# ev-hansen/Configurable-Spectrograms

Measured on NVIDIA B200. Metric: orbits/sec (whole box, device-timed), higher is better.
Workload: dtype f32

## Files before the change

configurable_spectrograms_b200/csrc/raster.cu:

```cuda
#include "common.cuh"

namespace {

constexpr int I_UNDER = 256, I_OVER = 257, I_BAD = 258;

template <typename T>
__device__ __forceinline__ T round_to(double v) {
  return (T)v;
}

template <typename T>
__device__ __forceinline__ T log10_d(T v);
template <>
__device__ __forceinline__ float log10_d<float>(float v) {
  return (float)log10((double)v);
}
template <>
__device__ __forceinline__ double log10_d<double>(double v) {
  return log10(v);
}

template <typename T>
__device__ __forceinline__ T substitute(T v, const csg_panel_norm& nm, bool log_scale) {
  if (log_scale) {
    if (!is_finite(v) || v <= T(0)) v = (T)nm.fill_lo;
  } else {
    if (is_nan(v)) v = (T)nm.fill_lo;
    if (v == (T)(-CUDART_INF)) v = (T)nm.fill_lo;
    if (v == (T)CUDART_INF) v = (T)nm.fill_hi;
  }
  return v;
}

template <typename T>
__device__ __forceinline__ int cmap_index_direct(T v, const csg_panel_norm& nm, bool log_scale) {
  if (nm.degenerate == 1) return 0;
  T x;
  if (log_scale) {
    const T t = log10_d<T>(v);
    x = (T)((double)t - nm.t_vmin);
    x = (T)((double)x / nm.t_range);
    if (!is_finite(x)) return I_BAD;
  } else {
    x = (T)((double)v - nm.t_vmin);
    x = (T)((double)x / nm.t_range);
  }
  T xa = mul_rn(x, T(256));
  if (xa == T(256)) xa = T(255);
  if (is_nan(xa)) return I_BAD;
  if (xa < T(0)) return I_UNDER;
  if (xa >= T(256)) return I_OVER;
  return (int)xa;
}

template <typename T>
__device__ __forceinline__ int monotone_code(T v, const csg_panel_norm& nm, bool log_scale) {
  const int idx = cmap_index_direct<T>(v, nm, log_scale);
  return idx == I_UNDER ? -1 : (idx == I_OVER ? 256 : idx);
}

constexpr int kThr = 257;
constexpr int kThrPitch = 264;

template <typename T>
__global__ void __launch_bounds__(288)
    panel_threshold_kernel(const csg_panel* __restrict__ panels, const csg_panel_norm* __restrict__ norms, int n_panels,
                           T* __restrict__ thresholds) {
  typedef typename Key<T>::U U;
  const int pi = blockIdx.x;
  const int k = threadIdx.x;
  if (k >= kThr) return;
  const csg_panel_norm nm = norms[pi];
  T* out = thresholds + (size_t)pi * kThrPitch;
  if (nm.status != CSG_NORM_OK || nm.degenerate != 0) {
    out[k] = (T)CUDART_INF;
    return;
  }
  const bool log_scale = panels[pi].log_scale != 0;
  const U dom_lo = log_scale ? Key<T>::key((T)0) + 1 : Key<T>::key((T)(-CUDART_INF));
  const U dom_hi = log_scale ? Key<T>::key((T)CUDART_INF) - 1 : Key<T>::key((T)CUDART_INF);
  auto code = [&](U key) { return monotone_code<T>(Key<T>::val(key), nm, log_scale); };
  const double frac = (double)k / 256.0;
  double guess = log_scale ? exp10(nm.t_vmin + frac * nm.t_range) : nm.t_vmin + frac * nm.t_range;
  T gT = (T)guess;
  if (is_nan(gT)) gT = T(1);
  U g = Key<T>::key(gT);
  if (g < dom_lo) g = dom_lo;
  if (g > dom_hi) g = dom_hi;
  U lo, hi;
  U step = 2;
  bool found = true;
  if (code(g) >= k) {
    hi = g;
    while (true) {
      if (hi == dom_lo) {
        lo = hi;
        break;
      }
      lo = (hi - dom_lo > step) ? hi - step : dom_lo;
      if (code(lo) < k) break;
      hi = lo;
      step <<= 2;
    }
  } else {
    lo = g;
    while (true) {
      if (lo == dom_hi) {
        found = false;
        break;
      }
      hi = (dom_hi - lo > step) ? lo + step : dom_hi;
      if (code(hi) >= k) break;
      lo = hi;
      step <<= 2;
    }
  }
  if (!found) {
    out[k] = (T)CUDART_INF;
    return;
  }
  while (hi - lo > 1) {
    const U mid = lo + ((hi - lo) >> 1);
    if (code(mid) >= k)
      hi = mid;
    else
      lo = mid;
  }
  out[k] = Key<T>::val(hi);
}

template <typename T>
__global__ void panel_prepare_kernel(const csg_panel* __restrict__ panels, int n_panels,
                                     const csg_region_stats* __restrict__ stats, const double* __restrict__ zvals,
                                     csg_panel_norm* __restrict__ norms) {
  const int i = blockIdx.x * blockDim.x + threadIdx.x;
  if (i >= n_panels) return;
  const csg_panel p = panels[i];
  const csg_region_stats own = stats[p.stat_region >= 0 ? p.stat_region : p.region];
  const csg_region_stats pct = stats[p.pct_region >= 0 ? p.pct_region : p.region];
  const double given_lo = (p.zmin_slot >= 0 && zvals) ? zvals[p.zmin_slot] : p.z_min;
  const double given_hi = (p.zmax_slot >= 0 && zvals) ? zvals[p.zmax_slot] : p.z_max;
  double zmin = is_nan(given_lo) ? pct.p_lo : given_lo;
  double zmax = is_nan(given_hi) ? pct.p_hi : given_hi;
  csg_panel_norm nm;
  nm.status = CSG_NORM_OK;
  nm.degenerate = 0;
  nm.c0 = nm.c1 = 0.f;
  if (p.log_scale) {
    const double safe = own.n_pos > 0 ? own.min_pos : 1e-10;
    double m = zmin;
    if (safe > m) m = safe;
    if (1e-10 > m) m = 1e-10;
    zmin = m;
    nm.vmin = zmin, nm.vmax = zmax;
    nm.fill_lo = (double)(T)zmin;
    nm.fill_hi = (double)(T)zmax;
    if (zmin > zmax) {
      nm.status = CSG_NORM_VMIN_GT_VMAX;
    } else if (zmin == zmax) {
      nm.degenerate = 1;
    }
    const double tlo = log10(zmin), thi = log10(zmax);
    nm.t_vmin = tlo;
    nm.t_range = thi - tlo;
    if (nm.status == CSG_NORM_OK && !nm.degenerate && !(is_finite(tlo) && is_finite(thi)))
      nm.status = CSG_NORM_INVALID;
  } else {
    nm.fill_lo = (double)(T)zmin;
    nm.fill_hi = (double)(T)zmax;
    if (!(is_finite(zmin) && is_finite(zmax) && zmax > zmin)) {
      double lo = CUDART_INF, hi = -CUDART_INF;
      bool any = false;
      if (own.fin_min <= own.fin_max) {
        lo = own.fin_min, hi = own.fin_max, any = true;
      }
      if ((own.n_nan > 0 || own.n_neginf > 0) && !is_nan(nm.fill_lo)) {
        lo = fmin(lo, nm.fill_lo), hi = fmax(hi, nm.fill_lo), any = true;
      }
      if (own.n_posinf > 0 && !is_nan(nm.fill_hi)) {
        lo = fmin(lo, nm.fill_hi), hi = fmax(hi, nm.fill_hi), any = true;
      }
      zmin = any ? lo : CUDART_NAN;
      zmax = any ? hi : CUDART_NAN;
    }
    nm.vmin = zmin, nm.vmax = zmax;
    nm.t_vmin = zmin;
    nm.t_range = zmax - zmin;
    if (zmin == zmax)
      nm.degenerate = 1;
    else if (zmin > zmax)
      nm.status = CSG_NORM_VMIN_GT_VMAX;
    else if (is_nan(zmin) || is_nan(zmax))
      nm.degenerate = 2;
  }
  nm.c1 = p.log_scale ? (float)(256.0 * 0.30102999566398120 / nm.t_range) : (float)(256.0 / nm.t_range);
  nm.c0 = (float)(-256.0 * nm.t_vmin / nm.t_range) + 1.0f;
  norms[i] = nm;
}

constexpr int kRasterThreads = 512;
constexpr int kPixPerThread = 16;
constexpr int kPixPerBlock = kRasterThreads * kPixPerThread;
constexpr int kRows = kThr + 2;
constexpr int kLutRows = 260;

__device__ __forceinline__ float fast_log2(float x) {
  float r;
  asm("lg2.approx.ftz.f32 %0, %1;" : "=f"(r) : "f"(x));
  return r;
}

__device__ __forceinline__ void lds(float& v, unsigned addr) { asm volatile("ld.shared.f32 %0, [%1];" : "=f"(v) : "r"(addr)); }
__device__ __forceinline__ void lds(double& v, unsigned addr) { asm volatile("ld.shared.f64 %0, [%1];" : "=d"(v) : "r"(addr)); }

template <typename T>
__device__ __noinline__ int recount(T v, int n, unsigned thr_col) {
  if (is_nan(v)) return 258;
  auto thr_at = [&](int row) -> T {
    T t;
    lds(t, thr_col + (unsigned)row * (32u * (unsigned)sizeof(T)));
    return t;
  };
  while (n > 0 && !(thr_at(n) <= v)) --n;
  while (n < kThr && thr_at(n + 1) <= v) ++n;
  return n;
}

template <bool B>
struct Flag {
  static constexpr bool value = B;
};

template <typename T>
constexpr size_t raster_smem_bytes() {
  return (size_t)kLutRows * 32 * sizeof(uint32_t) + (size_t)kRows * 32 * sizeof(T);
}

template <typename T>
__global__ void __launch_bounds__(kRasterThreads, sizeof(T) == 4 ? 3 : 2)
    rasterise_kernel(const T* __restrict__ mats, const csg_region* __restrict__ regions,
                     const int32_t* __restrict__ pool, const csg_panel* __restrict__ panels,
                     const csg_panel_norm* __restrict__ norms, int chunk_offset, int n_chunks,
                     const int32_t* __restrict__ block_panel, const T* __restrict__ thresholds,
                     const uint32_t* __restrict__ lut, uint32_t* __restrict__ rgba, uint16_t* __restrict__ index) {
  extern __shared__ __align__(16) unsigned char s_raw[];
  T* s_thr = reinterpret_cast<T*>(s_raw);
  uint32_t* s_lut = reinterpret_cast<uint32_t*>(s_raw + (size_t)kRows * 32 * sizeof(T));

  const int tid = threadIdx.x, lane = tid & 31;
  const int per = (n_chunks + (int)gridDim.x - 1) / (int)gridDim.x;
  const int c_begin = (int)blockIdx.x * per, c_end = min(n_chunks, c_begin + per);
  if (c_begin >= c_end) return;
  for (int w = tid; w < kLutRows * 32; w += kRasterThreads) {
    const int n = w >> 5;
    const int idx = n == 0 ? I_UNDER : (n == kThr ? I_OVER : (n <= 256 ? n - 1 : I_BAD));
    s_lut[w] = (lut && n < 259) ? __ldg(lut + idx) : 0u;
  }
  unsigned thr_col = (unsigned)__cvta_generic_to_shared(s_thr + lane);
  unsigned lut_col = (unsigned)__cvta_generic_to_shared(s_lut + lane);
  asm volatile("" : "+r"(thr_col), "+r"(lut_col));
  auto thr_at = [&](int row) -> T {
    T v;
    lds(v, thr_col + (unsigned)row * (32u * (unsigned)sizeof(T)));
    return v;
  };
  auto lut_at = [&](int row) -> uint32_t {
    uint32_t v;
    asm volatile("ld.shared.u32 %0, [%1];" : "=r"(v) : "r"(lut_col + (unsigned)row * 128u));
    return v;
  };

  int cur_panel = -1;
  bool skip = false, log_scale = false;
  int degenerate = 0;
  unsigned nt = 1, n_pix = 0;
  int first_block = 0, ld = 0, t0 = 0, rows_off = -1;
  long long out_off = 0;
  float c1 = 0.f, c0 = 0.f;
  T fill_lo = T(0), fill_hi = T(0);
  const T* mat = mats;
  const int32_t *cols = pool, *rows = pool;
  bool in_vec = false;

  for (int chunk = c_begin; chunk < c_end; ++chunk) {
    const int blk = chunk + chunk_offset;
    const int pi = __ldg(block_panel + blk);
    if (pi != cur_panel) {
      cur_panel = pi;
      const csg_panel* pn = panels + pi;
      const csg_region* rg = regions + __ldg(&pn->region);
      const csg_panel_norm* nm = norms + pi;
      skip = __ldg(&nm->status) != CSG_NORM_OK;
      degenerate = __ldg(&nm->degenerate);
      log_scale = __ldg(&pn->log_scale) != 0;
      nt = (unsigned)__ldg(&rg->nt);
      n_pix = (unsigned)__ldg(&rg->ne) * nt;
      first_block = __ldg(&pn->first_block);
      out_off = __ldg(&pn->out_off);
      c1 = __ldg(&nm->c1), c0 = __ldg(&nm->c0);
      fill_lo = (T)__ldg(&nm->fill_lo), fill_hi = (T)__ldg(&nm->fill_hi);
      mat = mats + __ldg(&rg->mat_off);
      cols = pool + __ldg(&rg->cols_off);
      rows_off = __ldg(&rg->rows_off);
      rows = pool + (rows_off < 0 ? 0 : rows_off);
      ld = __ldg(&rg->ld), t0 = __ldg(&rg->t0);
      in_vec = sizeof(T) == 4 && rows_off < 0 && (ld & 3) == 0 && (__ldg(&rg->mat_off) & 3) == 0 &&
               (reinterpret_cast<uintptr_t>(mats) & 15) == 0;
      __syncthreads();
      if (!skip && degenerate == 0) {
        const T* thr = thresholds + (size_t)pi * kThrPitch;
        for (int w = tid; w < kRows * 32; w += kRasterThreads) {
          const int k = (w >> 5) - 1;
          s_thr[w] = k < 0 ? (T)(-CUDART_INF) : (k >= kThr ? (T)CUDART_INF : __ldg(thr + k));
        }
      }
      __syncthreads();
    }
    if (skip) continue;
    const unsigned first = (unsigned)(blk - first_block) * kPixPerBlock;
    const unsigned last = first + kPixPerBlock < n_pix ? first + kPixPerBlock : n_pix;
    uint32_t* out_rgba = rgba ? rgba + out_off : nullptr;
    uint16_t* out_idx = index ? index + out_off : nullptr;
    if (degenerate != 0) {
      const int idx = degenerate == 1 ? 0 : I_BAD;
      const int row = degenerate == 1 ? 1 : 258;
      for (unsigned i = first + tid; i < last; i += kRasterThreads) {
        if (out_rgba) out_rgba[i] = lut_at(row);
        if (out_idx) out_idx[i] = (uint16_t)idx;
      }
      continue;
    }

    auto substituted = [&](T v, auto log_c) -> T {
      constexpr bool LOG = decltype(log_c)::value;
      if (LOG) return (v > T(0)) & is_finite(v) ? v : fill_lo;
      v = (is_nan(v) || v == (T)(-CUDART_INF)) ? fill_lo : v;
      return (v == (T)CUDART_INF) ? fill_hi : v;
    };
    auto guess = [&](T v, auto log_c, bool& ok) -> int {
      constexpr bool LOG = decltype(log_c)::value;
      const float fv = (float)v;
      float gf = __fmaf_rn(LOG ? fast_log2(fv) : fv, c1, c0);
      gf = fminf(fmaxf(gf, 0.f), (float)kThr);
      const int n = (int)gf;
      const unsigned row = thr_col + (unsigned)n * (32u * (unsigned)sizeof(T));
      T lo_thr, hi_thr;
      lds(lo_thr, row);
      lds(hi_thr, row + 32u * (unsigned)sizeof(T));
      ok = ok & (lo_thr <= v) & !(hi_thr <= v);
      return n;
    };
    auto to_count = [&](T raw, auto log_c) -> int {
      const T v = substituted(raw, log_c);
      bool ok = true;
      const int n = guess(v, log_c, ok);
      return ok ? n : recount<T>(v, n, thr_col);
    };
    auto count_to_index = [](int n) -> int { return n == 0 ? I_UNDER : (n == kThr ? I_OVER : (n == 258 ? I_BAD : n - 1)); };

    const bool out_vec = (out_off & 3) == 0 && (!out_rgba || (reinterpret_cast<uintptr_t>(rgba) & 15) == 0) &&
                         (!out_idx || (reinterpret_cast<uintptr_t>(index) & 7) == 0);
    auto pixels = [&](auto log_c, auto rowlist_c, auto rgba_c, auto idx_c, auto vec_c) {
      constexpr bool ROWLIST = decltype(rowlist_c)::value;
      constexpr bool RGBA = decltype(rgba_c)::value, INDEX = decltype(idx_c)::value, VEC = decltype(vec_c)::value;
      constexpr unsigned G = 4, STEP = G * kRasterThreads;
      unsigned i = first + G * tid;
      unsigned j = i / nt, tt = i - j * nt;
      const unsigned dq = STEP / nt, dr = STEP - dq * nt;
      auto address = [&](unsigned jj, unsigned t) -> unsigned {
        return (unsigned)(__ldg(cols + jj) * ld + (ROWLIST ? __ldg(rows + t) : t0 + (int)t));
      };
      auto load4 = [&](unsigned jj, unsigned t, T* v) {
        if (t + (G - 1) < nt) {
          const unsigned a0 = address(jj, t);
          if (!ROWLIST && in_vec && (a0 & 3u) == 0) {
            if constexpr (sizeof(T) == 4) {
              const float4 q = __ldg(reinterpret_cast<const float4*>(mat + a0));
              v[0] = q.x, v[1] = q.y, v[2] = q.z, v[3] = q.w;
            }
          } else if (!ROWLIST) {
#pragma unroll
            for (unsigned u = 0; u < G; ++u) v[u] = __ldg(mat + a0 + u);
          } else {
            const unsigned c = (unsigned)(__ldg(cols + jj) * ld);
#pragma unroll
            for (unsigned u = 0; u < G; ++u) v[u] = __ldg(mat + c + __ldg(rows + t + u));
          }
        } else {
#pragma unroll
          for (unsigned u = 0; u < G; ++u) {
            v[u] = __ldg(mat + address(jj, t));
            if (++t == nt) t = 0, ++jj;
          }
        }
      };
      auto store4 = [&](unsigned at, const int* n) {
        if constexpr (RGBA) {
          if constexpr (VEC)
            *reinterpret_cast<uint4*>(out_rgba + at) = make_uint4(lut_at(n[0]), lut_at(n[1]), lut_at(n[2]), lut_at(n[3]));
          else {
#pragma unroll
            for (unsigned u = 0; u < G; ++u) out_rgba[at + u] = lut_at(n[u]);
          }
        }
        if constexpr (INDEX) {
          int idx[G];
#pragma unroll
          for (unsigned u = 0; u < G; ++u) idx[u] = count_to_index(n[u]);
          if constexpr (VEC)
            *reinterpret_cast<uint2*>(out_idx + at) =
                make_uint2((unsigned)idx[0] | ((unsigned)idx[1] << 16), (unsigned)idx[2] | ((unsigned)idx[3] << 16));
          else {
#pragma unroll
            for (unsigned u = 0; u < G; ++u) out_idx[at + u] = (uint16_t)idx[u];
          }
        }
      };
      auto advance = [&]() {
        i += STEP, j += dq, tt += dr;
        if (tt >= nt) tt -= nt, ++j;
      };
      auto classify_store = [&](unsigned at, T* v) {
        int x[G];
        bool ok = true;
#pragma unroll
        for (unsigned u = 0; u < G; ++u) {
          v[u] = substituted(v[u], log_c);
          x[u] = guess(v[u], log_c, ok);
        }
        if (!ok) {
#pragma unroll
          for (unsigned u = 0; u < G; ++u) x[u] = recount<T>(v[u], x[u], thr_col);
        }
        store4(at, x);
      };
      while (i + STEP + (G - 1) < last) {
        T a[G], b[G];
        const unsigned ia = i;
        load4(j, tt, a);
        advance();
        const unsigned ib = i;
        load4(j, tt, b);
        advance();
        classify_store(ia, a);
        classify_store(ib, b);
      }
      while (i + (G - 1) < last) {
        T cur[G];
        load4(j, tt, cur);
        classify_store(i, cur);
        advance();
      }
      if (i < last) {
        unsigned jj = j, t = tt;
        for (unsigned p = i; p < last; ++p) {
          const int n = to_count(__ldg(mat + address(jj, t)), log_c);
          if constexpr (RGBA) out_rgba[p] = lut_at(n);
          if constexpr (INDEX) out_idx[p] = (uint16_t)count_to_index(n);
          if (++t == nt) t = 0, ++jj;
        }
      }
    };
    auto by_output = [&](auto log_c, auto rowlist_c) {
      if (out_rgba && !out_idx && out_vec)
        pixels(log_c, rowlist_c, Flag<true>{}, Flag<false>{}, Flag<true>{});
      else if (out_rgba && out_idx && out_vec)
        pixels(log_c, rowlist_c, Flag<true>{}, Flag<true>{}, Flag<true>{});
      else if (out_rgba && out_idx)
        pixels(log_c, rowlist_c, Flag<true>{}, Flag<true>{}, Flag<false>{});
      else if (out_rgba)
        pixels(log_c, rowlist_c, Flag<true>{}, Flag<false>{}, Flag<false>{});
      else if (out_idx)
        pixels(log_c, rowlist_c, Flag<false>{}, Flag<true>{}, Flag<false>{});
    };
    if (log_scale) {
      if (rows_off < 0)
        by_output(Flag<true>{}, Flag<false>{});
      else
        by_output(Flag<true>{}, Flag<true>{});
    } else {
      if (rows_off < 0)
        by_output(Flag<false>{}, Flag<false>{});
      else
        by_output(Flag<false>{}, Flag<true>{});
    }
  }
}

}

extern "C" {

int32_t csg_raster_blocks(int32_t ne, int32_t nt) {
  if (ne <= 0 || nt <= 0) return 0;
  return (int32_t)(((long long)ne * nt + kPixPerBlock - 1) / kPixPerBlock);
}

size_t csg_threshold_bytes(int n_panels, int dtype) {
  return (size_t)(n_panels > 0 ? n_panels : 0) * kThrPitch * (dtype == CSG_F64 ? 8 : 4);
}

int csg_panel_prepare(csg_ctx* ctx, const csg_panel* d_panels, int n_panels, const csg_region* d_regions,
                      const csg_region_stats* d_stats, int dtype, const double* d_zvals, csg_panel_norm* d_norms,
                      void* d_thresholds) {
  (void)d_regions;
  if (!ctx) return CSG_ERR_ARG;
  if (n_panels <= 0) return CSG_OK;
  if (!d_panels || !d_stats || !d_norms || !d_thresholds) return csg_fail(ctx, CSG_ERR_ARG, "NULL argument");
  const int blocks = (n_panels + 127) / 128;
  if (dtype == CSG_F32) {
    panel_prepare_kernel<float><<<blocks, 128, 0, ctx->stream>>>(d_panels, n_panels, d_stats, d_zvals, d_norms);
    CSG_LAUNCH_CHECK(ctx, "panel_prepare_kernel");
    panel_threshold_kernel<float><<<n_panels, 288, 0, ctx->stream>>>(d_panels, d_norms, n_panels, (float*)d_thresholds);
  } else if (dtype == CSG_F64) {
    panel_prepare_kernel<double><<<blocks, 128, 0, ctx->stream>>>(d_panels, n_panels, d_stats, d_zvals, d_norms);
    CSG_LAUNCH_CHECK(ctx, "panel_prepare_kernel");
    panel_threshold_kernel<double><<<n_panels, 288, 0, ctx->stream>>>(d_panels, d_norms, n_panels, (double*)d_thresholds);
  } else {
    return csg_fail(ctx, CSG_ERR_ARG, "bad dtype %d", dtype);
  }
  CSG_LAUNCH_CHECK(ctx, "panel_threshold_kernel");
  return CSG_OK;
}

int csg_rasterise(csg_ctx* ctx, const void* d_mats, int dtype, const csg_region* d_regions,
                  const int32_t* d_index_pool, const csg_panel* d_panels, const csg_panel_norm* d_norms,
                  const void* d_thresholds, int n_panels, int total_blocks, int block_offset,
                  const int32_t* d_block_panel, const uint8_t* d_lut, uint8_t* d_rgba, uint16_t* d_index) {
  if (!ctx) return CSG_ERR_ARG;
  if (n_panels <= 0 || total_blocks <= 0) return CSG_OK;
  if (!d_mats || !d_regions || !d_index_pool || !d_panels || !d_norms || !d_thresholds || !d_block_panel)
    return csg_fail(ctx, CSG_ERR_ARG, "NULL argument");
  if (d_rgba && !d_lut) return csg_fail(ctx, CSG_ERR_ARG, "d_rgba requested without d_lut");
  static bool configured_dev[64] = {false};
  bool& configured = configured_dev[ctx->device & 63];
  if (!configured) {
    CSG_CUDA(ctx, cudaFuncSetAttribute(rasterise_kernel<float>, cudaFuncAttributeMaxDynamicSharedMemorySize,
                                       (int)raster_smem_bytes<float>()));
    CSG_CUDA(ctx, cudaFuncSetAttribute(rasterise_kernel<double>, cudaFuncAttributeMaxDynamicSharedMemorySize,
                                       (int)raster_smem_bytes<double>()));
    configured = true;
  }
  int per_sm = dtype == CSG_F32 ? 3 : 2;
  if (ctx->raster_blocks_per_sm > 0 && ctx->raster_blocks_per_sm < per_sm) per_sm = ctx->raster_blocks_per_sm;
  int grid = ctx->sm_count * per_sm;
  if (grid > total_blocks) grid = total_blocks;
  if (dtype == CSG_F32)
    rasterise_kernel<float><<<grid, kRasterThreads, raster_smem_bytes<float>(), ctx->stream>>>(
        (const float*)d_mats, d_regions, d_index_pool, d_panels, d_norms, block_offset, total_blocks, d_block_panel,
        (const float*)d_thresholds, (const uint32_t*)d_lut, (uint32_t*)d_rgba, d_index);
  else if (dtype == CSG_F64)
    rasterise_kernel<double><<<grid, kRasterThreads, raster_smem_bytes<double>(), ctx->stream>>>(
        (const double*)d_mats, d_regions, d_index_pool, d_panels, d_norms, block_offset, total_blocks, d_block_panel,
        (const double*)d_thresholds, (const uint32_t*)d_lut, (uint32_t*)d_rgba, d_index);
  else
    return csg_fail(ctx, CSG_ERR_ARG, "bad dtype %d", dtype);
  CSG_LAUNCH_CHECK(ctx, "rasterise_kernel");
  return CSG_OK;
}

int csg_rasterise_blocks_per_sm(csg_ctx* ctx, int blocks_per_sm) {
  if (!ctx || blocks_per_sm < 0) return CSG_ERR_ARG;
  ctx->raster_blocks_per_sm = blocks_per_sm;
  return CSG_OK;
}

}
```

Measured before the change: 42450.

## Pipeline raster loads with cp.async ring and cache row bases in shared memory

Adds a 4-stage cp.async shared-memory ring for f32 rasterisation on panels without row lists, so global loads of matrix values overlap with classification and stores. Precomputes per-column row base offsets into a shared table, and processes a whole panel segment per block iteration instead of reloading panel state for each chunk. Also caps registers with __maxnreg__, drops f32 blocks per SM from 3 to 2, and guards the threshold search step against overflow. The extra shared memory and the lower occupancy may offset the latency-hiding gain.

```diff
diff --git a/configurable_spectrograms_b200/csrc/raster.cu b/configurable_spectrograms_b200/csrc/raster.cu
--- a/configurable_spectrograms_b200/csrc/raster.cu
+++ b/configurable_spectrograms_b200/csrc/raster.cu
@@ -89,6 +89,7 @@
   if (g > dom_hi) g = dom_hi;
   U lo, hi;
   U step = 2;
+  auto grow = [](U s) -> U { return s > (~U(0) >> 2) ? ~U(0) : U(s << 2); };
   bool found = true;
   if (code(g) >= k) {
     hi = g;
@@ -100,7 +101,7 @@
       lo = (hi - dom_lo > step) ? hi - step : dom_lo;
       if (code(lo) < k) break;
       hi = lo;
-      step <<= 2;
+      step = grow(step);
     }
   } else {
     lo = g;
@@ -112,7 +113,7 @@
       hi = (dom_hi - lo > step) ? lo + step : dom_hi;
       if (code(hi) >= k) break;
       lo = hi;
-      step <<= 2;
+      step = grow(step);
     }
   }
   if (!found) {
@@ -203,6 +204,8 @@
 constexpr int kPixPerBlock = kRasterThreads * kPixPerThread;
 constexpr int kRows = kThr + 2;
 constexpr int kLutRows = 260;
+constexpr int kRowTable = 256;
+constexpr int kStages = 4;
 
 __device__ __forceinline__ float fast_log2(float x) {
   float r;
@@ -231,13 +234,36 @@
   static constexpr bool value = B;
 };
 
+enum CellPath { kDirect, kRowList, kStaged };
+template <int P>
+struct Path {
+  static constexpr int value = P;
+};
+
+__device__ __forceinline__ void cp_async16(unsigned dst, const void* src) {
+  asm volatile("cp.async.cg.shared.global [%0], [%1], 16;" ::"r"(dst), "l"(src) : "memory");
+}
+__device__ __forceinline__ void cp_async4(unsigned dst, const void* src) {
+  asm volatile("cp.async.ca.shared.global [%0], [%1], 4;" ::"r"(dst), "l"(src) : "memory");
+}
+__device__ __forceinline__ void cp_async4x4(unsigned dst, const void* src) {
+  asm volatile(
+      "cp.async.ca.shared.global [%0], [%1], 4;\n\t"
+      "cp.async.ca.shared.global [%0+4], [%1+4], 4;\n\t"
+      "cp.async.ca.shared.global [%0+8], [%1+8], 4;\n\t"
+      "cp.async.ca.shared.global [%0+12], [%1+12], 4;" ::"r"(dst),
+      "l"(src)
+      : "memory");
+}
+
 template <typename T>
 constexpr size_t raster_smem_bytes() {
-  return (size_t)kLutRows * 32 * sizeof(uint32_t) + (size_t)kRows * 32 * sizeof(T);
-}
-
-template <typename T>
-__global__ void __launch_bounds__(kRasterThreads, sizeof(T) == 4 ? 3 : 2)
+  return (size_t)kLutRows * 32 * sizeof(uint32_t) + (size_t)kRows * 32 * sizeof(T) + (size_t)kRowTable * sizeof(int32_t) +
+         (sizeof(T) == 4 ? (size_t)kStages * kRasterThreads * 16 : 0);
+}
+
+template <typename T>
+__global__ void __maxnreg__(sizeof(T) == 4 ? 48 : 64)
     rasterise_kernel(const T* __restrict__ mats, const csg_region* __restrict__ regions,
                      const int32_t* __restrict__ pool, const csg_panel* __restrict__ panels,
                      const csg_panel_norm* __restrict__ norms, int chunk_offset, int n_chunks,
@@ -246,6 +272,8 @@
   extern __shared__ __align__(16) unsigned char s_raw[];
   T* s_thr = reinterpret_cast<T*>(s_raw);
   uint32_t* s_lut = reinterpret_cast<uint32_t*>(s_raw + (size_t)kRows * 32 * sizeof(T));
+  int32_t* s_row = reinterpret_cast<int32_t*>(s_lut + kLutRows * 32);
+  unsigned char* s_ring = reinterpret_cast<unsigned char*>(s_row + kRowTable);
 
   const int tid = threadIdx.x, lane = tid & 31;
   const int per = (n_chunks + (int)gridDim.x - 1) / (int)gridDim.x;
@@ -258,7 +286,9 @@
   }
   unsigned thr_col = (unsigned)__cvta_generic_to_shared(s_thr + lane);
   unsigned lut_col = (unsigned)__cvta_generic_to_shared(s_lut + lane);
-  asm volatile("" : "+r"(thr_col), "+r"(lut_col));
+  unsigned ring_col = (unsigned)__cvta_generic_to_shared(s_ring + 16 * tid);
+  unsigned row_tab_at = (unsigned)__cvta_generic_to_shared(s_row);
+  asm volatile("" : "+r"(thr_col), "+r"(lut_col), "+r"(ring_col), "+r"(row_tab_at));
   auto thr_at = [&](int row) -> T {
     T v;
     lds(v, thr_col + (unsigned)row * (32u * (unsigned)sizeof(T)));
@@ -270,55 +300,46 @@
     return v;
   };
 
-  int cur_panel = -1;
-  bool skip = false, log_scale = false;
-  int degenerate = 0;
-  unsigned nt = 1, n_pix = 0;
-  int first_block = 0, ld = 0, t0 = 0, rows_off = -1;
-  long long out_off = 0;
-  float c1 = 0.f, c0 = 0.f;
-  T fill_lo = T(0), fill_hi = T(0);
-  const T* mat = mats;
-  const int32_t *cols = pool, *rows = pool;
-  bool in_vec = false;
-
-  for (int chunk = c_begin; chunk < c_end; ++chunk) {
+  for (int chunk = c_begin; chunk < c_end;) {
     const int blk = chunk + chunk_offset;
     const int pi = __ldg(block_panel + blk);
-    if (pi != cur_panel) {
-      cur_panel = pi;
-      const csg_panel* pn = panels + pi;
-      const csg_region* rg = regions + __ldg(&pn->region);
-      const csg_panel_norm* nm = norms + pi;
-      skip = __ldg(&nm->status) != CSG_NORM_OK;
-      degenerate = __ldg(&nm->degenerate);
-      log_scale = __ldg(&pn->log_scale) != 0;
-      nt = (unsigned)__ldg(&rg->nt);
-      n_pix = (unsigned)__ldg(&rg->ne) * nt;
-      first_block = __ldg(&pn->first_block);
-      out_off = __ldg(&pn->out_off);
-      c1 = __ldg(&nm->c1), c0 = __ldg(&nm->c0);
-      fill_lo = (T)__ldg(&nm->fill_lo), fill_hi = (T)__ldg(&nm->fill_hi);
-      mat = mats + __ldg(&rg->mat_off);
-      cols = pool + __ldg(&rg->cols_off);
-      rows_off = __ldg(&rg->rows_off);
-      rows = pool + (rows_off < 0 ? 0 : rows_off);
-      ld = __ldg(&rg->ld), t0 = __ldg(&rg->t0);
-      in_vec = sizeof(T) == 4 && rows_off < 0 && (ld & 3) == 0 && (__ldg(&rg->mat_off) & 3) == 0 &&
-               (reinterpret_cast<uintptr_t>(mats) & 15) == 0;
-      __syncthreads();
-      if (!skip && degenerate == 0) {
-        const T* thr = thresholds + (size_t)pi * kThrPitch;
-        for (int w = tid; w < kRows * 32; w += kRasterThreads) {
-          const int k = (w >> 5) - 1;
-          s_thr[w] = k < 0 ? (T)(-CUDART_INF) : (k >= kThr ? (T)CUDART_INF : __ldg(thr + k));
-        }
-      }
-      __syncthreads();
+    const csg_panel* pn = panels + pi;
+    const csg_region* rg = regions + __ldg(&pn->region);
+    const csg_panel_norm* nm = norms + pi;
+    const bool skip = __ldg(&nm->status) != CSG_NORM_OK;
+    const int degenerate = __ldg(&nm->degenerate);
+    const bool log_scale = __ldg(&pn->log_scale) != 0;
+    const unsigned ne = (unsigned)__ldg(&rg->ne), nt = (unsigned)__ldg(&rg->nt);
+    const unsigned n_pix = ne * nt;
+    const int first_block = __ldg(&pn->first_block);
+    const long long out_off = __ldg(&pn->out_off);
+    const float c1 = __ldg(&nm->c1), c0 = __ldg(&nm->c0);
+    const T fill_lo = (T)__ldg(&nm->fill_lo), fill_hi = (T)__ldg(&nm->fill_hi);
+    const T* mat = mats + __ldg(&rg->mat_off);
+    const int32_t* cols = pool + __ldg(&rg->cols_off);
+    const int rows_off = __ldg(&rg->rows_off);
+    const int32_t* rows = pool + (rows_off < 0 ? 0 : rows_off);
+    const int ld = __ldg(&rg->ld), t0 = __ldg(&rg->t0);
+    const bool in_vec = rows_off < 0 && (ld & 3) == 0 && (__ldg(&rg->mat_off) & 3) == 0 &&
+                        (reinterpret_cast<uintptr_t>(mats) & 15) == 0;
+    const bool row_tab = rows_off < 0 && ne <= (unsigned)kRowTable;
+    const int seg_end = min(c_end, first_block + (int)((n_pix + kPixPerBlock - 1) / kPixPerBlock) - chunk_offset);
+    const unsigned first = (unsigned)(blk - first_block) * kPixPerBlock;
+    const unsigned seg_pix = (unsigned)(seg_end + chunk_offset - first_block) * kPixPerBlock;
+    const unsigned last = seg_pix < n_pix ? seg_pix : n_pix;
+    chunk = seg_end;
+    if (skip) continue;
+    __syncthreads();
+    if (degenerate == 0) {
+      const T* thr = thresholds + (size_t)pi * kThrPitch;
+      for (int w = tid; w < kRows * 32; w += kRasterThreads) {
+        const int k = (w >> 5) - 1;
+        s_thr[w] = k < 0 ? (T)(-CUDART_INF) : (k >= kThr ? (T)CUDART_INF : __ldg(thr + k));
+      }
+      if (row_tab)
+        for (unsigned w = tid; w < ne; w += kRasterThreads) s_row[w] = __ldg(cols + w) * ld + t0;
     }
-    if (skip) continue;
-    const unsigned first = (unsigned)(blk - first_block) * kPixPerBlock;
-    const unsigned last = first + kPixPerBlock < n_pix ? first + kPixPerBlock : n_pix;
+    __syncthreads();
     uint32_t* out_rgba = rgba ? rgba + out_off : nullptr;
     uint16_t* out_idx = index ? index + out_off : nullptr;
     if (degenerate != 0) {
@@ -360,25 +381,27 @@
 
     const bool out_vec = (out_off & 3) == 0 && (!out_rgba || (reinterpret_cast<uintptr_t>(rgba) & 15) == 0) &&
                          (!out_idx || (reinterpret_cast<uintptr_t>(index) & 7) == 0);
-    auto pixels = [&](auto log_c, auto rowlist_c, auto rgba_c, auto idx_c, auto vec_c) {
-      constexpr bool ROWLIST = decltype(rowlist_c)::value;
+    auto pixels = [&](auto log_c, auto path_c, auto rgba_c, auto idx_c, auto vec_c) {
+      constexpr bool ROWLIST = decltype(path_c)::value == kRowList, STAGED = decltype(path_c)::value == kStaged;
       constexpr bool RGBA = decltype(rgba_c)::value, INDEX = decltype(idx_c)::value, VEC = decltype(vec_c)::value;
       constexpr unsigned G = 4, STEP = G * kRasterThreads;
       unsigned i = first + G * tid;
       unsigned j = i / nt, tt = i - j * nt;
       const unsigned dq = STEP / nt, dr = STEP - dq * nt;
+      auto row_base = [&](unsigned jj) -> unsigned {
+        if (!STAGED && !row_tab) return (unsigned)(__ldg(cols + jj) * ld + t0);
+        unsigned b;
+        asm volatile("ld.shared.u32 %0, [%1];" : "=r"(b) : "r"(row_tab_at + 4u * jj));
+        return b;
+      };
       auto address = [&](unsigned jj, unsigned t) -> unsigned {
-        return (unsigned)(__ldg(cols + jj) * ld + (ROWLIST ? __ldg(rows + t) : t0 + (int)t));
+        if constexpr (ROWLIST) return (unsigned)(__ldg(cols + jj) * ld + __ldg(rows + t));
+        return row_base(jj) + t;
       };
       auto load4 = [&](unsigned jj, unsigned t, T* v) {
         if (t + (G - 1) < nt) {
-          const unsigned a0 = address(jj, t);
-          if (!ROWLIST && in_vec && (a0 & 3u) == 0) {
-            if constexpr (sizeof(T) == 4) {
-              const float4 q = __ldg(reinterpret_cast<const float4*>(mat + a0));
-              v[0] = q.x, v[1] = q.y, v[2] = q.z, v[3] = q.w;
-            }
-          } else if (!ROWLIST) {
+          if constexpr (!ROWLIST) {
+            const unsigned a0 = address(jj, t);
 #pragma unroll
             for (unsigned u = 0; u < G; ++u) v[u] = __ldg(mat + a0 + u);
           } else {
@@ -434,22 +457,63 @@
         }
         store4(at, x);
       };
-      while (i + STEP + (G - 1) < last) {
-        T a[G], b[G];
-        const unsigned ia = i;
-        load4(j, tt, a);
-        advance();
-        const unsigned ib = i;
-        load4(j, tt, b);
-        advance();
-        classify_store(ia, a);
-        classify_store(ib, b);
-      }
-      while (i + (G - 1) < last) {
-        T cur[G];
-        load4(j, tt, cur);
-        classify_store(i, cur);
-        advance();
+      if constexpr (STAGED) {
+        unsigned ii = i;
+        auto issue = [&](unsigned stage) {
+          if (ii + (G - 1) < last) {
+            const unsigned dst = ring_col + stage * (16u * kRasterThreads);
+            if (tt + (G - 1) < nt) {
+              const unsigned a0 = row_base(j) + tt;
+              if (in_vec && (a0 & 3u) == 0)
+                cp_async16(dst, mat + a0);
+              else
+                cp_async4x4(dst, mat + a0);
+            } else {
+              unsigned jj = j, t = tt;
+#pragma unroll
+              for (unsigned u = 0; u < G; ++u) {
+                cp_async4(dst + 4u * u, mat + row_base(jj) + t);
+                if (++t == nt) t = 0, ++jj;
+              }
+            }
+          }
+          asm volatile("cp.async.commit_group;" ::: "memory");
+          ii += STEP, j += dq, tt += dr;
+          if (tt >= nt) tt -= nt, ++j;
+        };
+#pragma unroll
+        for (unsigned st = 0; st + 1 < (unsigned)kStages; ++st) issue(st);
+        for (unsigned st = 0; i + (G - 1) < last; i += STEP, st = (st + 1) & (kStages - 1)) {
+          issue((st + kStages - 1) & (kStages - 1));
+          asm volatile("cp.async.wait_group %0;" ::"n"(kStages - 1) : "memory");
+          unsigned r[G];
+          asm volatile("ld.shared.v4.u32 {%0,%1,%2,%3}, [%4];"
+                       : "=r"(r[0]), "=r"(r[1]), "=r"(r[2]), "=r"(r[3])
+                       : "r"(ring_col + st * (16u * kRasterThreads)));
+          T v[G];
+#pragma unroll
+          for (unsigned u = 0; u < G; ++u) v[u] = __uint_as_float(r[u]);
+          classify_store(i, v);
+        }
+        j = i / nt, tt = i - j * nt;
+      } else {
+        while (i + STEP + (G - 1) < last) {
+          T a[G], b[G];
+          const unsigned ia = i;
+          load4(j, tt, a);
+          advance();
+          const unsigned ib = i;
+          load4(j, tt, b);
+          advance();
+          classify_store(ia, a);
+          classify_store(ib, b);
+        }
+        while (i + (G - 1) < last) {
+          T cur[G];
+          load4(j, tt, cur);
+          classify_store(i, cur);
+          advance();
+        }
       }
       if (i < last) {
         unsigned jj = j, t = tt;
@@ -461,29 +525,30 @@
         }
       }
     };
-    auto by_output = [&](auto log_c, auto rowlist_c) {
+    auto by_output = [&](auto log_c, auto path_c) {
       if (out_rgba && !out_idx && out_vec)
-        pixels(log_c, rowlist_c, Flag<true>{}, Flag<false>{}, Flag<true>{});
+        pixels(log_c, path_c, Flag<true>{}, Flag<false>{}, Flag<true>{});
       else if (out_rgba && out_idx && out_vec)
-        pixels(log_c, rowlist_c, Flag<true>{}, Flag<true>{}, Flag<true>{});
+        pixels(log_c, path_c, Flag<true>{}, Flag<true>{}, Flag<true>{});
       else if (out_rgba && out_idx)
-        pixels(log_c, rowlist_c, Flag<true>{}, Flag<true>{}, Flag<false>{});
+        pixels(log_c, path_c, Flag<true>{}, Flag<true>{}, Flag<false>{});
       else if (out_rgba)
-        pixels(log_c, rowlist_c, Flag<true>{}, Flag<false>{}, Flag<false>{});
+        pixels(log_c, path_c, Flag<true>{}, Flag<false>{}, Flag<false>{});
       else if (out_idx)
-        pixels(log_c, rowlist_c, Flag<false>{}, Flag<true>{}, Flag<false>{});
+        pixels(log_c, path_c, Flag<false>{}, Flag<true>{}, Flag<false>{});
     };
-    if (log_scale) {
-      if (rows_off < 0)
-        by_output(Flag<true>{}, Flag<false>{});
+    auto by_scale = [&](auto path_c) {
+      if (log_scale)
+        by_output(Flag<true>{}, path_c);
       else
-        by_output(Flag<true>{}, Flag<true>{});
-    } else {
-      if (rows_off < 0)
-        by_output(Flag<false>{}, Flag<false>{});
-      else
-        by_output(Flag<false>{}, Flag<true>{});
-    }
+        by_output(Flag<false>{}, path_c);
+    };
+    if (rows_off >= 0)
+      by_scale(Path<kRowList>{});
+    else if (row_tab)
+      by_scale(Path<sizeof(T) == 4 ? kStaged : kDirect>{});
+    else
+      by_scale(Path<kDirect>{});
   }
 }
 
@@ -541,7 +606,7 @@
                                        (int)raster_smem_bytes<double>()));
     configured = true;
   }
-  int per_sm = dtype == CSG_F32 ? 3 : 2;
+  int per_sm = 2;
   if (ctx->raster_blocks_per_sm > 0 && ctx->raster_blocks_per_sm < per_sm) per_sm = ctx->raster_blocks_per_sm;
   int grid = ctx->sm_count * per_sm;
   if (grid > total_blocks) grid = total_blocks;
```

Measured after the change: 42710, median of 6. No clear change (+0.6%).
